# moddyz/stereo-to-multiview-cuda

Hardware: AMD Instinct MI355X
Metric: stereo->8-view frames/sec @1080p d=64; cost-agg HBM GB/s vs roofline (higher is better)
Workload: dtype f32; 1 GPU; 1920x1080 synthetic stereo frame, D=64, zd=32, full stereo->8-view frame: cost init + cross aggregation + WTA + DCC/IRV x5/bilateral + 6 DIBR views + interlacing, one frame per GPU per step; stages=3, usd=34, lsd=17, views=8, aggregation=matrix pipe (stm_kernels_aggm.hip)

## Files before the change

### stereo-to-multiview-cuda_amd/csrc/stm_kernels_aggm.hip

```cpp
#include "stm_hwin.h"

namespace stm {

typedef float f4 __attribute__((ext_vector_type(4)));

#define STM_MFMA16(m, b, acc, abid) __builtin_amdgcn_mfma_f32_16x16x1f32(m, b, acc, 2, abid, 0)
typedef float f16v __attribute__((ext_vector_type(16)));
typedef uint32_t u4v __attribute__((ext_vector_type(4)));
#define STM_MASKF(m) (__builtin_amdgcn_inverse_ballot_w64(m) ? 1.0f : 0.0f)
#define STM_BLOAD(rsrc, voff) __builtin_bit_cast(f4, __builtin_amdgcn_raw_buffer_load_b128(rsrc, voff, 0, 2))


template <int N> __device__ __forceinline__ float row_ror_f(float v)
{
    return __builtin_bit_cast(float, __builtin_amdgcn_update_dpp(0, __builtin_bit_cast(int, v), 0x120 + N, 0xf, 0xf, false));
}
template <int N> __device__ __forceinline__ int row_ror_i(int v) { return __builtin_amdgcn_update_dpp(0, v, 0x120 + N, 0xf, 0xf, false); }
__device__ __forceinline__ int wave_min_i(int v)
{
    v = min(v, row_ror_i<8>(v)); v = min(v, row_ror_i<4>(v)); v = min(v, row_ror_i<2>(v)); v = min(v, row_ror_i<1>(v));
    return min(min(__builtin_amdgcn_readlane(v, 0), __builtin_amdgcn_readlane(v, 16)),
               min(__builtin_amdgcn_readlane(v, 32), __builtin_amdgcn_readlane(v, 48)));
}
__device__ __forceinline__ int wave_max_i(int v)
// ... 370 lines not shown
                }
                int it = 1;
                for (; it + 2 <= n_it; it += 2) {
                    STM_HS_NEXT(ca)
                    STM_HS_MFMA(cb)
                    STM_HS_NEXT(cb)
                    STM_HS_MFMA(ca)
                }
                if (it < n_it) STM_HS_MFMA(cb)
#undef STM_HS_NEXT
#undef STM_HS_MFMA
            } else {
#pragma unroll
                for (int i = 0; i < 16; ++i) acc[i] = 0.f;
            }
            if (!WTA) {
#pragma unroll
                for (int cl = 0; cl < 4; ++cl) {
                    const f4 o = {acc[4 * cl], acc[4 * cl + 1], acc[4 * cl + 2], acc[4 * cl + 3]};
                    STM_BSTORE(rout[cl], (X0 >> 2) * 256 + l * 16, o);
                }
            } else {
                float bc[4];
                int bd[4];
#pragma unroll
                for (int i = 0; i < 4; ++i) { bc[i] = 3.402823466e+38f; bd[i] = 0; }
#pragma unroll
                for (int cl = 0; cl < 4; ++cl) {
                    const int d = (c0 + cl) * 16 + dd;
                    if (d < D) {
#pragma unroll
                        for (int i = 0; i < 4; ++i)
                            if (bc[i] > acc[4 * cl + i]) { bc[i] = acc[4 * cl + i]; bd[i] = d; }
                    }
                }
                const __amdgpu_buffer_rsrc_t rs = __builtin_amdgcn_make_buffer_rsrc((void *)(disp + row), 0, (uint32_t)W * 4u, 0x00020000);
#pragma unroll
                for (int i = 0; i < 4; ++i) {
                    const int bi = __builtin_bit_cast(int, bc[i]);
                    int m = bi;
                    m = min(m, row_ror_i<8>(m));
                    m = min(m, row_ror_i<4>(m));
                    m = min(m, row_ror_i<2>(m));
                    m = min(m, row_ror_i<1>(m));
                    int cand = (bi == m) ? bd[i] : 0x7fffffff;
                    cand = min(cand, row_ror_i<8>(cand));
                    cand = min(cand, row_ror_i<4>(cand));
                    cand = min(cand, row_ror_i<2>(cand));
                    cand = min(cand, row_ror_i<1>(cand));
                    if (ncs > 1) {
                        uint2 *slot = wb + (X0 - seg0 * TX + 4 * lb + i);
                        if (dd == 0) {
                            if (cs > 0) {
                                const uint2 pv = *slot;
                                if (!(m < (int)pv.x)) { m = (int)pv.x; cand = (int)pv.y; }
                            }
                            if (cs + 1 < ncs) *slot = make_uint2((uint32_t)m, (uint32_t)cand);
                        }
                        if (cs + 1 < ncs) continue;
                    }
                    __builtin_amdgcn_raw_buffer_store_b32(__builtin_bit_cast(uint32_t, (float)cand - (float)zd), rs,
                                                          dd == 0 ? (X0 + 4 * lb + i) * 4 : (int)0x7ffffff0, 0, 0);
                }
            }
        }
        __syncthreads();
        if (more) {
            int sl = slot0 + w;
            if (sl >= NJ) sl -= NJ;
#pragma unroll
            for (int k = 0; k < KP; ++k) tile[(k * NJ + sl) * 64 + l] = st[k];
            STM_HS_SN(sq + 1)
            slot0 += NW;
            if (slot0 >= NJ) slot0 -= NJ;
        }
        __syncthreads();
    }
  }
#undef STM_HS_LOAD
#undef STM_HS_ARMS
#undef STM_HS_SN
}

template <int NW>
__global__ __launch_bounds__(64 * NW, (2 * NW) / 4) void stm_k_pq_hc(PQViews v, int D, int zd, int H, int W, int G, int NC, int HG, int nseg,
                                                                     int spl, const float *__restrict__ lut_g, int pad, int dbg)
{
    constexpr int NT = 64 * NW, TX = 16 * NW, NEWPX = 16 * NW;
    extern __shared__ f4 lds4[];
    const int NG = 4 * NW + 2 * HG, NJ = NG >> 2;
    f4 *tile = lds4;
    uint32_t *sn = (uint32_t *)(tile + 4 * NG * 16);
    int2 *sg = (int2 *)(sn + TX);
    const int SO = NEWPX + 2 * pad;
    uint2 *s_own = (uint2 *)(sg + NW), *s_oth = s_own + 2 * NEWPX;
    float *s_lut_ad = (float *)(s_oth + 2 * SO), *s_lut_c = s_lut_ad + 768;
    const int tid = threadIdx.x, l = tid & 63, w = __builtin_amdgcn_readfirstlane(tid >> 6);
    const int lb = l >> 4, dd = l & 15;
    const int part = blockIdx.x % spl, rest = blockIdx.x / spl, y = rest % H, view = rest / H;
    const int seg_per = (nseg + spl - 1) / spl, seg0 = part * seg_per, seg1 = min(nseg, seg0 + seg_per);
    if (seg0 >= seg1) return;
    f4 *__restrict__ out = (f4 *)(view ? v.b[1] : v.b[0]);
    const u8 *__restrict__ armL = view ? v.armL[1] : v.armL[0], *__restrict__ armR = view ? v.armR[1] : v.armR[0];
    const uint32_t *__restrict__ pk_own = view ? v.pk[1] : v.pk[0], *__restrict__ pk_oth = view ? v.pk[0] : v.pk[1];
    const uint32_t *__restrict__ cen_own = view ? v.cen[1] : v.cen[0], *__restrict__ cen_oth = view ? v.cen[0] : v.cen[1];
    const int sgn = view ? -1 : 1;
    const size_t row = (size_t)y * W;
    const uint32_t rowbytes = (uint32_t)G * 256u;
    for (int i = tid; i < 768 + 65; i += NT) s_lut_ad[i] = lut_g[i];
    uint2 so = make_uint2(0, 0), sx = make_uint2(0, 0);
    int aLn = 0, aRn = 0;
    f4 cst[4];
  const int ncs = (NC + 3) >> 2;
  for (int cs = 0; cs < ncs; ++cs) {
    const int c0 = 4 * cs;
    __amdgpu_buffer_rsrc_t rout[4];
#pragma unroll
    for (int cl = 0; cl < 4; ++cl)
        rout[cl] = __builtin_amdgcn_make_buffer_rsrc((void *)(out + ((size_t)min(c0 + cl, NC - 1) * H + y) * G * 16), 0, c0 + cl < NC ? rowbytes : 0u, 0x00020000);
#define STM_HC_FETCH(A0)                                                                           \
    {                                                                                              \
        const int x0_ = 4 * ((A0) - HG);                                                           \
        if (tid < NEWPX) {                                                                         \
            const int gx = min(max(x0_ + tid, 0), W - 1);                                          \
            so = make_uint2(pk_own[row + gx], cen_own[row + gx]);                                  \
        }                                                                                          \
        if (tid < SO) {                                                                            \
            const int gx = min(max(x0_ - pad + tid, 0), W - 1);                                    \
            sx = make_uint2(pk_oth[row + gx], cen_oth[row + gx]);                                  \
        }                                                                                          \
    }
#define STM_HC_STAGE(B)                                            \
    {                                                              \
        if (tid < NEWPX) s_own[(B) * NEWPX + tid] = so;            \
        if (tid < SO) s_oth[(B) * SO + tid] = sx;                  \
    }
#define STM_HC_COSTS(B, A0)                                                                                               \
    {                                                                                                                     \
        const int gi = 4 * w + lb, x0g = 4 * ((A0) - HG + gi);                                                            \
        const uint2 *own = s_own + (B) * NEWPX + gi * 4;                                                                  \
        const uint2 o0 = own[0], o1 = own[1], o2 = own[2], o3 = own[3];                                                   \
        const bool in0 = x0g >= 0 && x0g < W, in1 = x0g + 1 >= 0 && x0g + 1 < W, in2 = x0g + 2 >= 0 && x0g + 2 < W,       \
                   in3 = x0g + 3 >= 0 && x0g + 3 < W;                                                                     \
         \
         \
        _Pragma("unroll") for (int cl = 0; cl < 4; ++cl) {                                                                \
            f4 val = {0.f, 0.f, 0.f, 0.f};                                                                                \
            if (c0 + cl < NC) {                                                                              \
                const int d = (c0 + cl) * 16 + dd;                   \
                const uint2 *oth = s_oth + (B) * SO + gi * 4 + sgn * (d - zd) + pad;                                      \
                const uint2 q0 = oth[0], q1 = oth[1], q2 = oth[2], q3 = oth[3];                                           \
                const float a0 = s_lut_ad[__builtin_amdgcn_sad_u8(o0.x, q0.x, 0u)], c0 = s_lut_c[hamdist_q1(o0.y, q0.y)]; \
                const float a1 = s_lut_ad[__builtin_amdgcn_sad_u8(o1.x, q1.x, 0u)], c1 = s_lut_c[hamdist_q1(o1.y, q1.y)]; \
                const float a2 = s_lut_ad[__builtin_amdgcn_sad_u8(o2.x, q2.x, 0u)], c2 = s_lut_c[hamdist_q1(o2.y, q2.y)]; \
                const float a3 = s_lut_ad[__builtin_amdgcn_sad_u8(o3.x, q3.x, 0u)], c3 = s_lut_c[hamdist_q1(o3.y, q3.y)]; \
                const bool dok = d < D;                                                                                   \
                val.x = (in0 && dok) ? a0 + c0 : 0.f;                                                                     \
                val.y = (in1 && dok) ? a1 + c1 : 0.f;                                                                     \
                val.z = (in2 && dok) ? a2 + c2 : 0.f;                                                                     \
                val.w = (in3 && dok) ? a3 + c3 : 0.f;                                                                     \
            }                                                                                                             \
            cst[cl] = val;                                                                                                \
        }                                                                                                                 \
    }
#define STM_HC_ARMS(S)                                                          \
    if (tid < TX) {                                                             \
        const int x = min((S) * TX + tid, W - 1);                               \
        aLn = armL[row + x];                                                    \
        aRn = armR[row + x];                                                    \
    }
#define STM_HC_SN(S)                                                                                                       \
    if (tid < TX) {                                                                                                        \
        const int x = (S) * TX + tid, org = (S) * TX - 4 * HG;                                                             \
         \
        const int srel_ = x < W ? x - aLn - org : x - org, nn_ = x < W ? aLn + aRn : 0;                                    \
        sn[tid] = (uint32_t)srel_ | ((uint32_t)nn_ << 16);                                                                 \
                           \
        int lo_ = nn_ ? (srel_ >> 2) : 0x7fffffff, hi_ = nn_ ? ((srel_ + nn_ + 3) >> 2) : -0x7fffffff;                     \
        lo_ = min(lo_, row_ror_i<8>(lo_)); lo_ = min(lo_, row_ror_i<4>(lo_)); lo_ = min(lo_, row_ror_i<2>(lo_)); lo_ = min(lo_, row_ror_i<1>(lo_)); \
        hi_ = max(hi_, row_ror_i<8>(hi_)); hi_ = max(hi_, row_ror_i<4>(hi_)); hi_ = max(hi_, row_ror_i<2>(hi_)); hi_ = max(hi_, row_ror_i<1>(hi_)); \
        if ((tid & 15) == 0) sg[tid >> 4] = make_int2(lo_, hi_ - lo_);                                                     \
    }
    for (int r0 = 0; r0 < NJ; r0 += NW) {
        const int a0 = 4 * NW * seg0 + 4 * r0;
        STM_HC_FETCH(a0)
        __syncthreads();
        STM_HC_STAGE(0)
        __syncthreads();
        if (r0 + w < NJ) {
            STM_HC_COSTS(0, a0)
#pragma unroll
            for (int k = 0; k < 4; ++k) tile[(k * NJ + (NW * seg0 + r0 + w) % NJ) * 64 + l] = cst[k];
        }
    }
    __syncthreads();
    {
        const int a1 = 4 * NW * (seg0 + 1) + NG - 4 * NW;
        STM_HC_FETCH(a1)
        STM_HC_STAGE((seg0 + 1) & 1)
        STM_HC_ARMS(seg0)
        STM_HC_SN(seg0)
    }
    __syncthreads();
    int slot0 = (NW * seg0) % NJ;
    for (int sq = seg0; sq < seg1; ++sq) {
        const int X0 = sq * TX + 16 * w;
        const bool more = sq + 1 < seg1;
        if (more) {
            STM_HC_FETCH(4 * NW * (sq + 2) + NG - 4 * NW)
            STM_HC_ARMS(sq + 1)
        }
        if (X0 < W) {
            const uint32_t e = sn[16 * w + dd];
            const int srel = (int)(e & 0xffffu), nn = (int)(e >> 16);
            const int2 sgw = sg[w];
            const int G0r = __builtin_amdgcn_readfirstlane(sgw.x);
            const int n_it = STM_DBG(dbg, 1) ? 0 : __builtin_amdgcn_readfirstlane(sgw.y);
            f16v acc;
            if (n_it > 0) {
                int gs = 4 * slot0 + G0r;
                if (gs >= NG) gs -= NG;
                const f4 *p = tile + (lb * NG + gs) * 16 + dd;
                int t = 4 * G0r + lb - srel;
#define STM_HS_NEXT(C)                                        \
    {                                                         \
        C = *p;                                               \
        p += 16;                                              \
        if (++gs == NG) { gs = 0; p -= NG * 16; }  \
    }
#define STM_HS_MFMA(C)                                                          \
    {                                                                           \
        const float m = ((unsigned)t < (unsigned)nn) ? 1.0f : 0.0f;             \
        t += 4;                                                                 \
        acc = STM_MFMA16(m, C.x, acc, 0);                                       \
        acc = STM_MFMA16(m, C.y, acc, 1);                                       \
        acc = STM_MFMA16(m, C.z, acc, 2);                                       \
        acc = STM_MFMA16(m, C.w, acc, 3);                                       \
    }
                f4 ca, cb;
                STM_HS_NEXT(ca)
                STM_HS_NEXT(cb)
                {
                    const float m = ((unsigned)t < (unsigned)nn) ? 1.0f : 0.0f;
                    t += 4;
                    const f16v z = {0.f, 0.f, 0.f, 0.f, 0.f, 0.f, 0.f, 0.f, 0.f, 0.f, 0.f, 0.f, 0.f, 0.f, 0.f, 0.f};
                    acc = STM_MFMA16(m, ca.x, z, 0);
                    acc = STM_MFMA16(m, ca.y, acc, 1);
                    acc = STM_MFMA16(m, ca.z, acc, 2);
                    acc = STM_MFMA16(m, ca.w, acc, 3);
                }
                int it = 1;
                for (; it + 2 <= n_it; it += 2) {
                    STM_HS_NEXT(ca)
                    STM_HS_MFMA(cb)
                    STM_HS_NEXT(cb)
                    STM_HS_MFMA(ca)
                }
                if (it < n_it) STM_HS_MFMA(cb)
#undef STM_HS_NEXT
#undef STM_HS_MFMA
            } else {
#pragma unroll
                for (int i = 0; i < 16; ++i) acc[i] = 0.f;
            }
#pragma unroll
            for (int cl = 0; cl < 4; ++cl) {
                const f4 o = {acc[4 * cl], acc[4 * cl + 1], acc[4 * cl + 2], acc[4 * cl + 3]};
                if (!STM_DBG(dbg, 4)) STM_BSTORE(rout[cl], (X0 >> 2) * 256 + l * 16, o);
            }
        }
        if (more) STM_HC_COSTS((sq + 1) & 1, 4 * NW * (sq + 1) + NG - 4 * NW)
        __syncthreads();
        if (more) {
            int sl = slot0 + w;
            if (sl >= NJ) sl -= NJ;
#pragma unroll
            for (int k = 0; k < 4; ++k) tile[(k * NJ + sl) * 64 + l] = cst[k];
            STM_HC_STAGE(sq & 1)
            STM_HC_SN(sq + 1)
            slot0 += NW;
            if (slot0 >= NJ) slot0 -= NJ;
        }
        __syncthreads();
    }
  }
#undef STM_HC_FETCH
#undef STM_HC_STAGE
#undef STM_HC_COSTS
#undef STM_HC_ARMS
#undef STM_HC_SN
}

constexpr int VT_EV = 2 * 255 + 32;
__global__ __launch_bounds__(256) void stm_k_vwin_table(PQViews v, uint32_t *__restrict__ tab, int rec, int H, int W, int G, int nT, int top)
{
    __shared__ unsigned long long ev_all[4][VT_EV];
    const int l = threadIdx.x & 63, wv = threadIdx.x >> 6, g = blockIdx.x * 4 + wv, u = blockIdx.y, view = blockIdx.z;
    if (g >= G) return;
    unsigned long long *ev = ev_all[wv];
    const u8 *__restrict__ armU = view ? v.armU[1] : v.armU[0], *__restrict__ armD = view ? v.armD[1] : v.armD[0];
    const int b = l >> 4, i = l & 15, y = u * 16 + i, x = 4 * g + b;
    int s0 = 0, nn = 0;
    if (y < H && x < W) {
        const int aU = armU[(size_t)y * W + x], aD = armD[(size_t)y * W + x];
        s0 = y - aU;
        nn = aU + aD;
    }
    vwin_build(tab + ((size_t)(view * nT + u) * G + g) * rec, ev, u, top, s0, nn);
}

typedef __attribute__((address_space(4))) const uint32_t ctab32;
typedef __attribute__((address_space(4))) const unsigned long long ctab64;
struct V12Quad { f4 c; unsigned long long m0, m1, m2, m3; };
struct V12Sweep {
    const f4 *p;
    ctab64 *mk;
    int qs, n_it;
    V12Quad A;
};
#define STM_V12_LOAD(S, Q, RQ)                                                      \
    {                                                                               \
        Q.c = *S.p;                                                                 \
        Q.m0 = S.mk[0]; Q.m1 = S.mk[1]; Q.m2 = S.mk[2]; Q.m3 = S.mk[3];             \
        S.p += 64; S.mk += 4;                                                       \
        if (++S.qs == RQ) { S.qs = 0; S.p -= RQ * 64; }                \
        asm volatile("" ::: "memory"); __builtin_amdgcn_sched_barrier(0);           \
    }
#define STM_V12_ARRIVED(Q) __builtin_amdgcn_sched_barrier(0); asm volatile("" : : "v"(Q.c), "s"(Q.m0), "s"(Q.m1), "s"(Q.m2), "s"(Q.m3) : "memory");
#define STM_V12_MFMA(Q)                                                                                            \
    {                                                                                                              \
        float a0 = STM_MASKF(Q.m0), a1 = STM_MASKF(Q.m1), a2 = STM_MASKF(Q.m2), a3 = STM_MASKF(Q.m3);              \
        asm volatile("" : "+v"(a0), "+v"(a1), "+v"(a2), "+v"(a3));  \
        acc = __builtin_amdgcn_mfma_f32_16x16x1f32(a0, Q.c.x, acc, 0, 0, 0);                                       \
        acc = __builtin_amdgcn_mfma_f32_16x16x1f32(a1, Q.c.y, acc, 0, 0, 0);                                       \
        acc = __builtin_amdgcn_mfma_f32_16x16x1f32(a2, Q.c.z, acc, 0, 0, 0);                                       \
        acc = __builtin_amdgcn_mfma_f32_16x16x1f32(a3, Q.c.w, acc, 0, 0, 0);                                       \
    }
__device__ __forceinline__ void v12t_begin(V12Sweep &S, const f4 *ring_l, int RQ, int slot0, int u4, ctab32 *r, int K0, int n_it)
{
    int qs = slot0 + ((K0 >> 2) - u4);
    if (qs < 0) qs += RQ;
    if (qs >= RQ) qs -= RQ;
    S.qs = qs;
    S.n_it = n_it;
    S.p = ring_l + qs * 64;
    S.mk = (ctab64 *)(r + 8);
    STM_V12_LOAD(S, S.A, RQ)
}
#define STM_V12_MFMA0(Q)                                                                                           \
    {                                                                                                              \
        float a0 = STM_MASKF(Q.m0), a1 = STM_MASKF(Q.m1), a2 = STM_MASKF(Q.m2), a3 = STM_MASKF(Q.m3);              \
        asm volatile("" : "+v"(a0), "+v"(a1), "+v"(a2), "+v"(a3));                                                 \
        const f16v z = {0.f, 0.f, 0.f, 0.f, 0.f, 0.f, 0.f, 0.f, 0.f, 0.f, 0.f, 0.f, 0.f, 0.f, 0.f, 0.f};           \
        acc = __builtin_amdgcn_mfma_f32_16x16x1f32(a0, Q.c.x, z, 0, 0, 0);                                         \
        acc = __builtin_amdgcn_mfma_f32_16x16x1f32(a1, Q.c.y, acc, 0, 0, 0);                                       \
        acc = __builtin_amdgcn_mfma_f32_16x16x1f32(a2, Q.c.z, acc, 0, 0, 0);                                       \
        acc = __builtin_amdgcn_mfma_f32_16x16x1f32(a3, Q.c.w, acc, 0, 0, 0);                                       \
    }
__device__ __forceinline__ f16v v12t_run(V12Sweep &S, int RQ)
{
    f16v acc;
    const int n_it = S.n_it;
    if (n_it == 0) {
#pragma unroll
        for (int i = 0; i < 16; ++i) acc[i] = 0.f;
        return acc;
    }
    V12Quad B;
    STM_V12_ARRIVED(S.A)
    STM_V12_LOAD(S, B, RQ)
    STM_V12_MFMA0(S.A)
    int it = 1;
    for (; it + 2 <= n_it; it += 2) {
// ... 147 lines not shown
static size_t v12t_smem(int usd)
{
    const int TS = 48, UQ = (usd + 3) & ~3, LAG = (UQ + TS - 1) / TS + 1;
    return (size_t)(TS + 2 * UQ + TS * (LAG + 1) + UQ) * 256;
}
bool aggm_supports(int usd, int H, int W)
{
    if (usd > 255) usd = 255;
    return usd >= 1 && v12t_smem(usd) <= 160 * 1024 && (unsigned long long)H * ((W + 3) / 4) * 256ull < (1ull << 31);
}

template <bool QUAD> __global__ __launch_bounds__(256) void stm_k_from_pq(const f4 *__restrict__ in, Vol out, int D, int H, int W, int G)
{
    const int t = blockIdx.x * 256 + threadIdx.x, y = blockIdx.y, c = blockIdx.z;
    const int g = t >> 2, q = 4 * c + (t & 3);
    if (g >= G || 4 * q >= D) return;
    const f4 *src = in + (((size_t)c * H + y) * G + g) * 16 + 4 * (t & 3);
    const f4 d0 = src[0], d1 = src[1], d2 = src[2], d3 = src[3];
#pragma unroll
    for (int k = 0; k < 4; ++k) {
        const int x = 4 * g + k;
        if (x < W) store_quad<QUAD, false>(out, q, D, (size_t)y * W + x, make_float4(d0[k], d1[k], d2[k], d3[k]));
    }
}
void launch_from_pq(const float *pq, Vol out, int D, int H, int W)
{
    const int G = (W + 3) / 4, NC = (D + 15) / 16;
    if (out.quad) STM_LAUNCH(stm_k_from_pq<true>, dim3(cdiv(4 * G, 256), H, NC), dim3(256), 0, stream(), (const f4 *)pq, out, D, H, W, G);
    else STM_LAUNCH(stm_k_from_pq<false>, dim3(cdiv(4 * G, 256), H, NC), dim3(256), 0, stream(), (const f4 *)pq, out, D, H, W, G);
    STM_CHECK_LAUNCH();
}

static void aggm_chain(PQViews &v, int nviews, bool from_costs, bool wta, const float *lut, int D, int zd, int H, int W, int usd,
                       uint32_t *htab_ready = nullptr, uint32_t *vtab_ready = nullptr)
{
    const int G = (W + 3) / 4, NC = (D + 15) / 16;
    if (usd > 255) usd = 255;
    constexpr int NW = 8;
    const int HG = ((usd + 3) / 4 + 2) & ~1, NG = 4 * NW + 2 * HG;
    const int nseg = cdiv(W, 16 * NW), nblk = ((nseg * H * nviews + 7) / 8) * 8;
    const size_t smem_h = (size_t)4 * NG * 256 + 16 * NW * 4;
    const int dbgh = timing_knobs();
    int pad = zd > D - 1 - zd ? zd : D - 1 - zd;
    pad = (pad < 0 ? 0 : pad) + 15;
    const size_t smem_cost = smem_h + (size_t)(4 * NG * 4 + 4 * pad + 768 + 72) * 4;
    const bool fuse_cost = from_costs && (agg_variant() / 1000000) % 10 != 1;
    const int spl = nseg > 24 ? cdiv(nseg, 16) : 1;
    const bool streaming = NG / 4 >= NW && (agg_variant() / 10) % 10 != 1 && (NC <= 4 || (agg_variant() / 10) % 10 != 2);
    constexpr int NTP = 3, TS = 16 * NTP;
    const int UQ = (usd + 3) & ~3, nT = (H + 15) / 16;
    const bool regs = aggv_supports(usd) && (agg_variant() / 10000000) % 10 != 1;
    const int rec = regs ? aggv_table_rec() : 8 + 8 * ((2 * usd + 21) / 4 + 2);
    const int LAG = (UQ + TS - 1) / TS + 1;
    const int RQ1 = (TS + 2 * UQ) / 4, RQ2 = (TS * (LAG + 1) + UQ) / 4;
    uint32_t *vtab = regs && vtab_ready ? vtab_ready : Workspace::get<uint32_t>((size_t)nviews * nT * G * rec);
    const bool hregs = wta && aggh_supports(usd, D) && (agg_variant() / 100000000) % 10 != 1;
    uint32_t *htab = !hregs ? nullptr : htab_ready ? htab_ready : Workspace::get<uint32_t>(aggh_table_dwords(nviews, H, W));
    {
        if (!(regs && vtab_ready)) {
            ProfScope p("pq_vtab");
            STM_LAUNCH(stm_k_vwin_table, dim3(cdiv(G, 4), nT, nviews), dim3(256), 0, stream(), v, vtab, rec, H, W, G, nT, regs ? aggv_table_top() : -1);
            STM_CHECK_LAUNCH();
        }
        if (hregs && !htab_ready) {
            ProfScope p("pq_htab");
            launch_hwin_table(v, nviews, htab, H, W);
        }
    }
    if (from_costs && !fuse_cost) {
        ProfScope p("pq_cost");
        const size_t smem = (size_t)(2 * PC_TX + 2 * (PC_TX + 2 * pad) + 768 + 72) * 4;
        allow_lds_m((const void *)stm_k_pq_cost, smem);
        STM_LAUNCH(stm_k_pq_cost, dim3(cdiv(W, PC_TX), H, nviews), dim3(PC_TX), smem, stream(), v, lut, D, zd, H, W, G, NC, pad);
        STM_CHECK_LAUNCH();
    }
    {
        ProfScope p("pq_h");
        constexpr int NWC = 12;
        const int NGc = 4 * NWC + 2 * HG;
        const size_t smem_c12 = (size_t)4 * NGc * 256 + 16 * NWC * 4 + (size_t)(4 * NGc * 4 + 4 * pad + 768 + 72) * 4;
        const size_t smem_hc = (size_t)4 * NGc * 256 + 16 * NWC * 4 + 8 * NWC + (size_t)(2 * 16 * NWC + 2 * (16 * NWC + 2 * pad)) * 8 + (768 + 72) * 4;
        const int nsegc = cdiv(W, 16 * NWC);
        const size_t smem_hc8 = (size_t)4 * NG * 256 + 16 * NW * 4 + 8 * NW + (size_t)(2 * 16 * NW + 2 * (16 * NW + 2 * pad)) * 8 + (768 + 72) * 4;
        const bool hc_ok = fuse_cost && (agg_variant() / 1000) % 10 == 0 && (NC <= 4 || (agg_variant() / 10) % 10 != 2);
        if (hc_ok && smem_hc <= 80 * 1024 && 16 * NWC + 2 * pad <= 64 * NWC) {
            const int splc = nsegc > 24 ? cdiv(nsegc, 16) : 1;
            allow_lds_m((const void *)stm_k_pq_hc<NWC>, smem_hc);
            STM_LAUNCH((stm_k_pq_hc<NWC>), dim3(nviews * H * splc), dim3(64 * NWC), smem_hc, stream(), v, D, zd, H, W, G, NC, HG, nsegc, splc, lut, pad, dbgh);
        } else if (hc_ok && smem_hc8 <= 80 * 1024 && 16 * NW + 2 * pad <= 64 * NW) {
            allow_lds_m((const void *)stm_k_pq_hc<NW>, smem_hc8);
            STM_LAUNCH((stm_k_pq_hc<NW>), dim3(nviews * H * spl), dim3(64 * NW), smem_hc8, stream(), v, D, zd, H, W, G, NC, HG, nseg, spl, lut, pad, dbgh);
        } else if (fuse_cost && smem_c12 <= 80 * 1024 && (agg_variant() / 1000) % 10 != 1) {
            const int nblkc = ((nsegc * H * nviews + 7) / 8) * 8;
            allow_lds_m((const void *)stm_k_pq_h<NWC, false, true>, smem_c12);
            STM_LAUNCH((stm_k_pq_h<NWC, false, true>), dim3(nblkc), dim3(64 * NWC), smem_c12, stream(), v, D, zd, H, W, G, NC, HG, nsegc, dbgh, lut, pad, nviews);
        } else if (fuse_cost) {
            allow_lds_m((const void *)stm_k_pq_h<NW, false, true>, smem_cost);
            STM_LAUNCH((stm_k_pq_h<NW, false, true>), dim3(nblk), dim3(64 * NW), smem_cost, stream(), v, D, zd, H, W, G, NC, HG, nseg, dbgh, lut, pad, nviews);
        } else if (streaming) {
            allow_lds_m((const void *)stm_k_pq_hs<NW, false>, smem_h);
            STM_LAUNCH((stm_k_pq_hs<NW, false>), dim3(nviews * H * spl), dim3(64 * NW), smem_h, stream(), v, D, zd, H, W, G, NC, HG, nseg, spl, dbgh);
        } else {
            allow_lds_m((const void *)stm_k_pq_h<NW, false, false>, smem_h);
            STM_LAUNCH((stm_k_pq_h<NW, false, false>), dim3(nblk), dim3(64 * NW), smem_h, stream(), v, D, zd, H, W, G, NC, HG, nseg, dbgh, lut, 0, nviews);
        }
        STM_CHECK_LAUNCH();
    }
    {
        ProfScope p("pq_v12");
        if (regs) {
            launch_pq_v12r(v, nviews, vtab, rec, H, W, G, NC);
        } else {
            const size_t smem = (size_t)(RQ1 + RQ2) * 1024;
            allow_lds_m((const void *)stm_k_pq_v12t<NTP>, smem);
            STM_LAUNCH(stm_k_pq_v12t<NTP>, dim3(G, NC, nviews), dim3(128 * NTP), smem, stream(), v, vtab, rec, H, W, G, NC, UQ, RQ1, RQ2, LAG, dbgh);
            STM_CHECK_LAUNCH();
        }
    }
    {
        ProfScope p("pq_hw");
        if (hregs) {
            launch_pq_hsr(v, nviews, htab, D, zd, H, W);
        } else if (streaming && !wta) {
            allow_lds_m((const void *)stm_k_pq_hs<NW, false>, smem_h);
            STM_LAUNCH((stm_k_pq_hs<NW, false>), dim3(nviews * H * spl), dim3(64 * NW), smem_h, stream(), v, D, zd, H, W, G, NC, HG, nseg, spl, dbgh);
        } else if (streaming) {
            const int splw = NC > 4 ? std::max(spl, cdiv(nseg * 16 * NW, 1920)) : spl;
            const size_t smem_w = smem_h + (NC > 4 ? (size_t)cdiv(nseg, splw) * 16 * NW * 8 : 0);
            allow_lds_m((const void *)stm_k_pq_hs<NW, true>, smem_w);
            STM_LAUNCH((stm_k_pq_hs<NW, true>), dim3(nviews * H * splw), dim3(64 * NW), smem_w, stream(), v, D, zd, H, W, G, NC, HG, nseg, splw, dbgh);
        } else if (!wta) {
            allow_lds_m((const void *)stm_k_pq_h<NW, false, false>, smem_h);
            STM_LAUNCH((stm_k_pq_h<NW, false, false>), dim3(nblk), dim3(64 * NW), smem_h, stream(), v, D, zd, H, W, G, NC, HG, nseg, dbgh, lut, 0, nviews);
        } else {
            allow_lds_m((const void *)stm_k_pq_h<NW, true, false>, smem_h);
            STM_LAUNCH((stm_k_pq_h<NW, true, false>), dim3(nblk), dim3(64 * NW), smem_h, stream(), v, D, zd, H, W, G, NC, HG, nseg, dbgh, lut, 0, nviews);
        }
        STM_CHECK_LAUNCH();
    }
}

size_t aggm_frame_vtab_dwords(int H, int W, int usd, int *rec, int *top)
{
    if (usd > 255) usd = 255;
    const bool regs = aggv_supports(usd) && (agg_variant() / 10000000) % 10 != 1;
    *rec = regs ? aggv_table_rec() : 0;
    *top = regs ? aggv_table_top() : -1;
    if (!regs || (agg_variant() / 1000000000) % 10 == 1) return 0;
    return (size_t)2 * ((H + 15) / 16) * ((W + 3) / 4) * *rec;
}
size_t aggm_frame_htab_dwords(int D, int H, int W, int usd, bool keep_volume)
{
    if (usd > 255) usd = 255;
    const bool hregs = !keep_volume && aggh_supports(usd, D) && (agg_variant() / 100000000) % 10 != 1;
    return hregs && (agg_variant() / 1000000000) % 10 != 1 ? aggh_table_dwords(2, H, W) : 0;
}
void launch_aggm_frame(const uint32_t *const *pk, const uint32_t *const *cen, const float *lut, float *const *vol_a, float *const *vol_b,
                       const u8 *const *armU, const u8 *const *armD, const u8 *const *armL, const u8 *const *armR, float *const *disp,
                       int D, int zd, int H, int W, int usd, bool keep_volume, uint32_t *htab_ready, uint32_t *vtab_ready)
{
    PQViews v;
    for (int i = 0; i < 2; ++i) {
        v.pk[i] = pk[i]; v.cen[i] = cen[i]; v.a[i] = vol_a[i]; v.b[i] = vol_b[i];
        v.armU[i] = armU[i]; v.armD[i] = armD[i]; v.armL[i] = armL[i]; v.armR[i] = armR[i]; v.disp[i] = disp[i];
    }
    aggm_chain(v, 2, true, !keep_volume, lut, D, zd, H, W, usd, htab_ready, vtab_ready);
}

static int vtab_rec(int usd)
{
    if (usd > 255) usd = 255;
    const bool regs = aggv_supports(usd) && (agg_variant() / 10000000) % 10 != 1;
    return regs ? aggv_table_rec() : 8 + 8 * ((2 * usd + 21) / 4 + 2);
}
// ... 29 lines not shown
```

Measured before the change: 624.2 frames/s.

## Share fused cost ring between left and right views in horizontal aggregation

Adds a kernel that computes matching costs once per row into a circular LDS ring buffer and runs both the left- and right-view horizontal cross aggregations from it. The right view reads the same costs at disparity-shifted offsets, so one block per row handles both views. This halves the cost computation and the pk/census loads compared with launching a block per view. In exchange it needs a much larger LDS allocation (up to 160 KB), which lowers occupancy, and it adds ring-wraparound indexing. It is taken by default when nviews==2, NC<=4 and the ring fits.

```diff
diff --git a/stereo-to-multiview-cuda_amd/csrc/stm_kernels_aggm.hip b/stereo-to-multiview-cuda_amd/csrc/stm_kernels_aggm.hip
--- a/stereo-to-multiview-cuda_amd/csrc/stm_kernels_aggm.hip
+++ b/stereo-to-multiview-cuda_amd/csrc/stm_kernels_aggm.hip
@@ -683,6 +683,242 @@
 #undef STM_HC_COSTS
 #undef STM_HC_ARMS
 #undef STM_HC_SN
+}
+
+constexpr int HC2_RP = 512;
+template <int NW>
+__global__ __launch_bounds__(64 * NW, NW / 4) void stm_k_pq_hc2(PQViews v, int D, int zd, int H, int W, int G, int NC, int HG, int nseg, int spl,
+                                                                const float *__restrict__ lut_g, int pad, int EXL, int EXR)
+{
+    constexpr int NT = 64 * NW, TX = 16 * NW, RP = HC2_RP;
+    extern __shared__ f4 lds4[];
+    float *ring = (float *)lds4;
+    uint32_t *sn = (uint32_t *)(ring + (RP + 4) * 64);
+    int2 *sg = (int2 *)(sn + 2 * TX);
+    const int SO = TX + 2 * pad;
+    uint2 *s_own = (uint2 *)(sg + 2 * NW), *s_oth = s_own + 2 * TX;
+    float *s_lut_ad = (float *)(s_oth + 2 * SO), *s_lut_c = s_lut_ad + 768;
+    const int tid = threadIdx.x, l = tid & 63, w = __builtin_amdgcn_readfirstlane(tid >> 6);
+    const int lb = l >> 4, dd = l & 15;
+    const int part = blockIdx.x % spl, y = blockIdx.x / spl;
+    const int seg_per = (nseg + spl - 1) / spl, seg0 = part * seg_per, seg1 = min(nseg, seg0 + seg_per);
+    if (seg0 >= seg1) return;
+    const int ROFF = 4 * HG + EXL, RN = TX + 8 * HG + EXL + EXR;
+    const int dl = min(l, 16 * NC - 1);
+    const bool dok = l < D;
+    const int vw = tid >= TX ? 1 : 0, tv = tid - vw * TX;
+    const u8 *__restrict__ armLv = vw ? v.armL[1] : v.armL[0], *__restrict__ armRv = vw ? v.armR[1] : v.armR[0];
+    const uint32_t *__restrict__ pkL = v.pk[0], *__restrict__ pkR = v.pk[1], *__restrict__ cenL = v.cen[0], *__restrict__ cenR = v.cen[1];
+    const size_t row = (size_t)y * W;
+    const uint32_t rowbytes = (uint32_t)G * 256u;
+    for (int i = tid; i < 768 + 65; i += NT) s_lut_ad[i] = lut_g[i];
+    __amdgpu_buffer_rsrc_t rout[2][4];
+#pragma unroll
+    for (int vv = 0; vv < 2; ++vv)
+#pragma unroll
+        for (int cl = 0; cl < 4; ++cl)
+            rout[vv][cl] = __builtin_amdgcn_make_buffer_rsrc((void *)((f4 *)(vv ? v.b[1] : v.b[0]) + ((size_t)min(cl, NC - 1) * H + y) * G * 16), 0,
+                                                             cl < NC ? rowbytes : 0u, 0x00020000);
+    uint2 so = make_uint2(0, 0), sx = make_uint2(0, 0);
+    int aLn = 0, aRn = 0;
+    f4 cst[4];
+#define STM_HC2_FETCH(P0)                                                                          \
+    {                                                                                              \
+        const int p0_ = (P0);                                                                      \
+        if (tid < TX) {                                                                            \
+            const int gx = min(max(p0_ + tid, 0), W - 1);                                          \
+            so = make_uint2(pkL[row + gx], cenL[row + gx]);                                        \
+        }                                                                                          \
+        if (tid < SO) {                                                                            \
+            const int gx = min(max(p0_ - pad + tid, 0), W - 1);                                    \
+            sx = make_uint2(pkR[row + gx], cenR[row + gx]);                                        \
+        }                                                                                          \
+    }
+#define STM_HC2_STAGE(B)                                           \
+    {                                                              \
+        if (tid < TX) s_own[(B) * TX + tid] = so;                  \
+        if (tid < SO) s_oth[(B) * SO + tid] = sx;                  \
+    }
+#define STM_HC2_COSTS(B)                                                                                                  \
+    {                                                                                                                     \
+        _Pragma("unroll") for (int k = 0; k < 4; ++k) {                                                                   \
+            const uint2 *own = s_own + (B) * TX + 16 * w + 4 * k;                                                         \
+            const uint2 o0 = own[0], o1 = own[1], o2 = own[2], o3 = own[3];                                               \
+            const uint2 *oth = s_oth + (B) * SO + 16 * w + 4 * k + dl - zd + pad;                                         \
+            const uint2 q0 = oth[0], q1 = oth[1], q2 = oth[2], q3 = oth[3];                                               \
+            const float a0 = s_lut_ad[__builtin_amdgcn_sad_u8(o0.x, q0.x, 0u)], c0 = s_lut_c[hamdist_q1(o0.y, q0.y)];     \
+            const float a1 = s_lut_ad[__builtin_amdgcn_sad_u8(o1.x, q1.x, 0u)], c1 = s_lut_c[hamdist_q1(o1.y, q1.y)];     \
+            const float a2 = s_lut_ad[__builtin_amdgcn_sad_u8(o2.x, q2.x, 0u)], c2 = s_lut_c[hamdist_q1(o2.y, q2.y)];     \
+            const float a3 = s_lut_ad[__builtin_amdgcn_sad_u8(o3.x, q3.x, 0u)], c3 = s_lut_c[hamdist_q1(o3.y, q3.y)];     \
+            cst[k].x = dok ? a0 + c0 : 0.f;                                                                               \
+            cst[k].y = dok ? a1 + c1 : 0.f;                                                                               \
+            cst[k].z = dok ? a2 + c2 : 0.f;                                                                               \
+            cst[k].w = dok ? a3 + c3 : 0.f;                                                                               \
+        }                                                                                                                 \
+    }
+#define STM_HC2_WRITE(P0, NV)                                                                      \
+    {                                                                                              \
+        _Pragma("unroll") for (int k = 0; k < 4; ++k) {                                            \
+            if (16 * w + 4 * k < (NV)) {                                              \
+                const int rpix = ((P0) + 16 * w + 4 * k + ROFF) & (RP - 1);                        \
+                float *dst = ring + rpix * 64 + l;                                                 \
+                dst[0] = cst[k].x; dst[64] = cst[k].y; dst[128] = cst[k].z; dst[192] = cst[k].w;   \
+                if (rpix == 0) {                                                                   \
+                    dst[RP * 64] = cst[k].x; dst[RP * 64 + 64] = cst[k].y; dst[RP * 64 + 128] = cst[k].z; \
+                }                                                                                  \
+            }                                                                                      \
+        }                                                                                          \
+    }
+#define STM_HC2_ARMS(S)                                                         \
+    if (tid < 2 * TX) {                                                         \
+        const int x = min((S) * TX + tv, W - 1);                                \
+        aLn = armLv[row + x];                                                   \
+        aRn = armRv[row + x];                                                   \
+    }
+#define STM_HC2_SN(S)                                                                                                      \
+    if (tid < 2 * TX) {                                                                                                    \
+        const int x = (S) * TX + tv, org = (S) * TX - 4 * HG;                                                              \
+         \
+        const int srel_ = x < W ? x - aLn - org : x - org, nn_ = x < W ? aLn + aRn : 0;                                    \
+        sn[tid] = (uint32_t)srel_ | ((uint32_t)nn_ << 16);                                                                 \
+                           \
+        int lo_ = nn_ ? (srel_ >> 2) : 0x7fffffff, hi_ = nn_ ? ((srel_ + nn_ + 3) >> 2) : -0x7fffffff;                     \
+        lo_ = min(lo_, row_ror_i<8>(lo_)); lo_ = min(lo_, row_ror_i<4>(lo_)); lo_ = min(lo_, row_ror_i<2>(lo_)); lo_ = min(lo_, row_ror_i<1>(lo_)); \
+        hi_ = max(hi_, row_ror_i<8>(hi_)); hi_ = max(hi_, row_ror_i<4>(hi_)); hi_ = max(hi_, row_ror_i<2>(hi_)); hi_ = max(hi_, row_ror_i<1>(hi_)); \
+        if ((tid & 15) == 0) sg[tid >> 4] = make_int2(lo_, hi_ - lo_);                                                     \
+    }
+    const int pbeg = seg0 * TX - ROFF;
+    for (int r0 = 0; r0 < RN; r0 += TX) {
+        STM_HC2_FETCH(pbeg + r0)
+        __syncthreads();
+        STM_HC2_STAGE(0)
+        __syncthreads();
+        STM_HC2_COSTS(0)
+        STM_HC2_WRITE(pbeg + r0, RN - r0)
+    }
+    __syncthreads();
+#define STM_HC2_PNEW(S) (((S) - 1) * TX - ROFF + RN)
+    {
+        STM_HC2_FETCH(STM_HC2_PNEW(seg0 + 1))
+        STM_HC2_STAGE((seg0 + 1) & 1)
+        STM_HC2_ARMS(seg0)
+        STM_HC2_SN(seg0)
+    }
+    __syncthreads();
+    const float *ringl = ring + l;
+    for (int sq = seg0; sq < seg1; ++sq) {
+        const int X0 = sq * TX + 16 * w;
+        const bool more = sq + 1 < seg1;
+        if (more) {
+            STM_HC2_FETCH(STM_HC2_PNEW(sq + 2))
+            STM_HC2_ARMS(sq + 1)
+        }
+        if (X0 < W) {
+#define STM_HS_MFMA(C)                                                          \
+    {                                                                           \
+        const float m = ((unsigned)t < (unsigned)nn) ? 1.0f : 0.0f;             \
+        t += 4;                                                                 \
+        acc = STM_MFMA16(m, C.x, acc, 0);                                       \
+        acc = STM_MFMA16(m, C.y, acc, 1);                                       \
+        acc = STM_MFMA16(m, C.z, acc, 2);                                       \
+        acc = STM_MFMA16(m, C.w, acc, 3);                                       \
+    }
+#define STM_HC2_SWEEP(VV)                                                                                                  \
+    {                                                                                                                      \
+        f4 ca, cb;                                                                                                         \
+        STM_HS_NEXT(ca)                                                                                                    \
+        STM_HS_NEXT(cb)                               \
+        {                        \
+            const float m = ((unsigned)t < (unsigned)nn) ? 1.0f : 0.0f;                                                    \
+            t += 4;                                                                                                        \
+            const f16v z = {0.f, 0.f, 0.f, 0.f, 0.f, 0.f, 0.f, 0.f, 0.f, 0.f, 0.f, 0.f, 0.f, 0.f, 0.f, 0.f};               \
+            acc = STM_MFMA16(m, ca.x, z, 0);                                                                               \
+            acc = STM_MFMA16(m, ca.y, acc, 1);                                                                             \
+            acc = STM_MFMA16(m, ca.z, acc, 2);                                                                             \
+            acc = STM_MFMA16(m, ca.w, acc, 3);                                                                             \
+        }                                                                                                                  \
+        int it = 1;                                                                                                        \
+        for (; it + 2 <= n_it; it += 2) {                                                                                  \
+            STM_HS_NEXT(ca)                                                                                                \
+            STM_HS_MFMA(cb)                                                                                                \
+            STM_HS_NEXT(cb)                          \
+            STM_HS_MFMA(ca)                                                                                                \
+        }                                                                                                                  \
+        if (it < n_it) STM_HS_MFMA(cb)                                                                                     \
+    }
+#define STM_HC2_STORE(VV)                                                                                                  \
+    _Pragma("unroll") for (int cl = 0; cl < 4; ++cl) {  \
+        const f4 o = {acc[4 * cl], acc[4 * cl + 1], acc[4 * cl + 2], acc[4 * cl + 3]};                                     \
+        STM_BSTORE(rout[VV][cl], (X0 >> 2) * 256 + l * 16, o);                                                             \
+    }
+            {
+                const uint32_t e = sn[16 * w + dd];
+                const int srel = (int)(e & 0xffffu), nn = (int)(e >> 16);
+                const int2 sgw = sg[w];
+                const int G0r = __builtin_amdgcn_readfirstlane(sgw.x);
+                const int n_it = __builtin_amdgcn_readfirstlane(sgw.y);
+                f16v acc;
+                if (n_it > 0) {
+                    int ri = (sq * TX + 4 * G0r + EXL) & (RP - 1);
+                    int t = 4 * G0r + lb - srel;
+#define STM_HS_NEXT(C)                                                                  \
+    {                                                                                   \
+        const float *p_ = ringl + ri * 64;                                              \
+        C.x = p_[0]; C.y = p_[64]; C.z = p_[128]; C.w = p_[192];                        \
+        ri = (ri + 4) & (RP - 1);                                                       \
+    }
+                    STM_HC2_SWEEP(0)
+#undef STM_HS_NEXT
+                } else {
+#pragma unroll
+                    for (int i = 0; i < 16; ++i) acc[i] = 0.f;
+                }
+                STM_HC2_STORE(0)
+            }
+            {
+                const uint32_t e = sn[TX + 16 * w + dd];
+                const int srel = (int)(e & 0xffffu), nn = (int)(e >> 16);
+                const int2 sgw = sg[NW + w];
+                const int G0r = __builtin_amdgcn_readfirstlane(sgw.x);
+                const int n_it = __builtin_amdgcn_readfirstlane(sgw.y);
+                f16v acc;
+                if (n_it > 0) {
+                    uint32_t ab = ((uint32_t)((sq * TX + 4 * G0r + EXL - (dl - zd)) & (RP - 1)) << 8) | ((uint32_t)l << 2);
+                    int t = 4 * G0r + lb - srel;
+#define STM_HS_NEXT(C)                                                                  \
+    {                                                                                   \
+        const float *p_ = (const float *)((const char *)ring + ab);                     \
+        C.x = p_[0]; C.y = p_[64]; C.z = p_[128]; C.w = p_[192];                        \
+        ab = (ab + 1024u) & (uint32_t)(RP * 256 - 1);                                   \
+    }
+                    STM_HC2_SWEEP(1)
+#undef STM_HS_NEXT
+                } else {
+#pragma unroll
+                    for (int i = 0; i < 16; ++i) acc[i] = 0.f;
+                }
+                STM_HC2_STORE(1)
+            }
+#undef STM_HS_MFMA
+#undef STM_HC2_SWEEP
+#undef STM_HC2_STORE
+        }
+        if (more) STM_HC2_COSTS((sq + 1) & 1)
+        __syncthreads();
+        if (more) {
+            STM_HC2_WRITE(STM_HC2_PNEW(sq + 1), TX)
+            STM_HC2_STAGE(sq & 1)
+            STM_HC2_SN(sq + 1)
+        }
+        __syncthreads();
+    }
+#undef STM_HC2_FETCH
+#undef STM_HC2_STAGE
+#undef STM_HC2_COSTS
+#undef STM_HC2_WRITE
+#undef STM_HC2_ARMS
+#undef STM_HC2_SN
+#undef STM_HC2_PNEW
 }
 
 constexpr int VT_EV = 2 * 255 + 32;
@@ -996,8 +1232,18 @@
         const size_t smem_hc = (size_t)4 * NGc * 256 + 16 * NWC * 4 + 8 * NWC + (size_t)(2 * 16 * NWC + 2 * (16 * NWC + 2 * pad)) * 8 + (768 + 72) * 4;
         const int nsegc = cdiv(W, 16 * NWC);
         const size_t smem_hc8 = (size_t)4 * NG * 256 + 16 * NW * 4 + 8 * NW + (size_t)(2 * 16 * NW + 2 * (16 * NW + 2 * pad)) * 8 + (768 + 72) * 4;
-        const bool hc_ok = fuse_cost && (agg_variant() / 1000) % 10 == 0 && (NC <= 4 || (agg_variant() / 10) % 10 != 2);
-        if (hc_ok && smem_hc <= 80 * 1024 && 16 * NWC + 2 * pad <= 64 * NWC) {
+        const int hv = (agg_variant() / 1000) % 10;
+        const bool hc_ok = fuse_cost && (hv == 0 || hv == 3) && (NC <= 4 || (agg_variant() / 10) % 10 != 2);
+        const int exl = (std::max(16 * NC - 1 - zd, 0) + 3) & ~3, exr = (std::max(zd, 0) + 3) & ~3;
+        const size_t smem_hc2 = (size_t)(HC2_RP + 4) * 256 + 2 * 16 * NWC * 4 + 2 * NWC * 8 + (size_t)(2 * 16 * NWC + 2 * (16 * NWC + 2 * pad)) * 8 + (768 + 72) * 4;
+        const bool hc2_ok = hc_ok && hv != 3 && nviews == 2 && NC <= 4 && zd >= 0 && 16 * NWC + 2 * pad <= 64 * NWC &&
+                            16 * NWC + 8 * HG + exl + exr <= HC2_RP && smem_hc2 <= 160 * 1024;
+        if (hc2_ok) {
+            ProfScope ps("hc_shared");
+            const int splc = nsegc > 24 ? cdiv(nsegc, 16) : 1;
+            allow_lds_m((const void *)stm_k_pq_hc2<NWC>, smem_hc2);
+            STM_LAUNCH((stm_k_pq_hc2<NWC>), dim3(H * splc), dim3(64 * NWC), smem_hc2, stream(), v, D, zd, H, W, G, NC, HG, nsegc, splc, lut, pad, exl, exr);
+        } else if (hc_ok && smem_hc <= 80 * 1024 && 16 * NWC + 2 * pad <= 64 * NWC) {
             const int splc = nsegc > 24 ? cdiv(nsegc, 16) : 1;
             allow_lds_m((const void *)stm_k_pq_hc<NWC>, smem_hc);
             STM_LAUNCH((stm_k_pq_hc<NWC>), dim3(nviews * H * splc), dim3(64 * NWC), smem_hc, stream(), v, D, zd, H, W, G, NC, HG, nsegc, splc, lut, pad, dbgh);
```

Measured after the change: 620.8 frames/s. No clear change (-0.5%).

## Specialize fused cost+horizontal-agg kernel with interior fast path and direct LDS addressing

Applied to the files above, without the earlier changes.

Splits the fused cost/horizontal aggregation kernel body into a template with a PARENT flag. The default variant gets an interior-tile cost path that skips per-pixel bounds checks and reads the LUTs through raw LDS addresses. The Hamming-LUT lookup is folded into popcount plus a bit offset. The MFMA feed loop now walks the ring-buffer tile pointer directly instead of going through the generic next macro. The old behaviour stays reachable as a selectable variant (hcv==3), at the cost of more code paths and address-space casts that depend on LUT layout assumptions.

```diff
diff --git a/stereo-to-multiview-cuda_amd/csrc/stm_kernels_aggm.hip b/stereo-to-multiview-cuda_amd/csrc/stm_kernels_aggm.hip
--- a/stereo-to-multiview-cuda_amd/csrc/stm_kernels_aggm.hip
+++ b/stereo-to-multiview-cuda_amd/csrc/stm_kernels_aggm.hip
@@ -476,9 +476,22 @@
 #undef STM_HS_SN
 }
 
-template <int NW>
-__global__ __launch_bounds__(64 * NW, (2 * NW) / 4) void stm_k_pq_hc(PQViews v, int D, int zd, int H, int W, int G, int NC, int HG, int nseg,
-                                                                     int spl, const float *__restrict__ lut_g, int pad, int dbg)
+typedef __attribute__((address_space(3))) const float hc_lds_cf;
+typedef uint32_t hc_u2 __attribute__((ext_vector_type(2)));
+typedef __attribute__((address_space(3))) const hc_u2 hc_lds_u2;
+__device__ __forceinline__ float hc_rho_c(uint32_t a, uint32_t b, uint32_t tab4)
+{
+    const uint32_t x = a ^ b;
+    return *(hc_lds_cf *)(uintptr_t)((((uint32_t)__popc(x) + tab4) << 2) + ((x >> 24) & 0x80u));
+}
+__device__ __forceinline__ float hc_rho_ad(uint32_t a, uint32_t b, uint32_t tab)
+{
+    return *(hc_lds_cf *)(uintptr_t)((__builtin_amdgcn_sad_u8(a, b, 0u) << 2) + tab);
+}
+
+template <int NW, bool PARENT>
+__device__ __forceinline__ void pq_hc_body(const PQViews &v, int D, int zd, int H, int W, int G, int NC, int HG, int nseg, int spl,
+                                           const float *__restrict__ lut_g, int pad, int dbg)
 {
     constexpr int NT = 64 * NW, TX = 16 * NW, NEWPX = 16 * NW;
     extern __shared__ f4 lds4[];
@@ -502,6 +515,8 @@
     const size_t row = (size_t)y * W;
     const uint32_t rowbytes = (uint32_t)G * 256u;
     for (int i = tid; i < 768 + 65; i += NT) s_lut_ad[i] = lut_g[i];
+    const uint32_t ad_lds = (uint32_t)(uintptr_t)(__attribute__((address_space(3))) float *)s_lut_ad;
+    const uint32_t c_lds4 = (uint32_t)(uintptr_t)(__attribute__((address_space(3))) float *)s_lut_c >> 2;
     uint2 so = make_uint2(0, 0), sx = make_uint2(0, 0);
     int aLn = 0, aRn = 0;
     f4 cst[4];
@@ -529,21 +544,21 @@
         if (tid < NEWPX) s_own[(B) * NEWPX + tid] = so;            \
         if (tid < SO) s_oth[(B) * SO + tid] = sx;                  \
     }
-#define STM_HC_COSTS(B, A0)                                                                                               \
+#define STM_HC_OTH(B)                                                                                                     \
+    const int d = (c0 + cl) * 16 + dd;                               \
+    const uint2 *oth = s_oth + (B) * SO + gi * 4 + sgn * (d - zd) + pad;                                                  \
+    const uint2 q0 = oth[0], q1 = oth[1], q2 = oth[2], q3 = oth[3];
+#define STM_HC_COSTS_EDGE(B, A0)                                                                                          \
     {                                                                                                                     \
         const int gi = 4 * w + lb, x0g = 4 * ((A0) - HG + gi);                                                            \
         const uint2 *own = s_own + (B) * NEWPX + gi * 4;                                                                  \
         const uint2 o0 = own[0], o1 = own[1], o2 = own[2], o3 = own[3];                                                   \
         const bool in0 = x0g >= 0 && x0g < W, in1 = x0g + 1 >= 0 && x0g + 1 < W, in2 = x0g + 2 >= 0 && x0g + 2 < W,       \
                    in3 = x0g + 3 >= 0 && x0g + 3 < W;                                                                     \
-         \
-         \
         _Pragma("unroll") for (int cl = 0; cl < 4; ++cl) {                                                                \
             f4 val = {0.f, 0.f, 0.f, 0.f};                                                                                \
             if (c0 + cl < NC) {                                                                              \
-                const int d = (c0 + cl) * 16 + dd;                   \
-                const uint2 *oth = s_oth + (B) * SO + gi * 4 + sgn * (d - zd) + pad;                                      \
-                const uint2 q0 = oth[0], q1 = oth[1], q2 = oth[2], q3 = oth[3];                                           \
+                STM_HC_OTH(B)                                                                                             \
                 const float a0 = s_lut_ad[__builtin_amdgcn_sad_u8(o0.x, q0.x, 0u)], c0 = s_lut_c[hamdist_q1(o0.y, q0.y)]; \
                 const float a1 = s_lut_ad[__builtin_amdgcn_sad_u8(o1.x, q1.x, 0u)], c1 = s_lut_c[hamdist_q1(o1.y, q1.y)]; \
                 const float a2 = s_lut_ad[__builtin_amdgcn_sad_u8(o2.x, q2.x, 0u)], c2 = s_lut_c[hamdist_q1(o2.y, q2.y)]; \
@@ -556,6 +571,48 @@
             }                                                                                                             \
             cst[cl] = val;                                                                                                \
         }                                                                                                                 \
+    }
+#define STM_HC_SUMS(CL)                                                                                                   \
+    {                                                                                                                     \
+         \
+        hc_lds_u2 *oth = (hc_lds_u2 *)(uintptr_t)(oth0 + (uint32_t)((CL) * 128 * sgn));                                   \
+        const hc_u2 q0 = oth[0], q1 = oth[1], q2 = oth[2], q3 = oth[3];                                                   \
+        cst[CL].x = hc_rho_ad(o0.x, q0.x, ad_lds) + hc_rho_c(o0.y, q0.y, c_lds4);                                         \
+        cst[CL].y = hc_rho_ad(o1.x, q1.x, ad_lds) + hc_rho_c(o1.y, q1.y, c_lds4);                                         \
+        cst[CL].z = hc_rho_ad(o2.x, q2.x, ad_lds) + hc_rho_c(o2.y, q2.y, c_lds4);                                         \
+        cst[CL].w = hc_rho_ad(o3.x, q3.x, ad_lds) + hc_rho_c(o3.y, q3.y, c_lds4);                                         \
+    }
+#define STM_HC_COSTS_IN(B, A0)                                                                                            \
+    {                                                                                                                     \
+        const int gi = 4 * w + lb;                                                                                        \
+        const uint2 *own = s_own + (B) * NEWPX + gi * 4;                                                                  \
+        const uint2 o0 = own[0], o1 = own[1], o2 = own[2], o3 = own[3];                                                   \
+         \
+         \
+        uint32_t oth0 = (uint32_t)(uintptr_t)(hc_lds_u2 *)(s_oth + (B) * SO + gi * 4 + sgn * (c0 * 16 + dd - zd) + pad); \
+        asm("" : "+v"(oth0));                                                                                             \
+        if ((c0 + 4) * 16 <= D) {                                       \
+            STM_HC_SUMS(0) STM_HC_SUMS(1) STM_HC_SUMS(2) STM_HC_SUMS(3)                                                   \
+        } else {                                                                                                          \
+            _Pragma("unroll") for (int cl = 0; cl < 4; ++cl) {                                                            \
+                if (c0 + cl < NC) {                                                                          \
+                    STM_HC_SUMS(cl)                                                                                       \
+                    if ((c0 + cl) * 16 + 16 > D) {                                        \
+                        const bool dok = (c0 + cl) * 16 + dd < D;                                                         \
+                        cst[cl].x = dok ? cst[cl].x : 0.f; cst[cl].y = dok ? cst[cl].y : 0.f;                             \
+                        cst[cl].z = dok ? cst[cl].z : 0.f; cst[cl].w = dok ? cst[cl].w : 0.f;                             \
+                    }                                                                                                     \
+                } else {                                                                                                  \
+                    cst[cl] = f4{0.f, 0.f, 0.f, 0.f};                                                                     \
+                }                                                                                                         \
+            }                                                                                                             \
+        }                                                                                                                 \
+    }
+#define STM_HC_COSTS(B, A0)                                                                                               \
+    {                                                                                                                     \
+        const int xw_ = 4 * ((A0) - HG + 4 * w);                           \
+        if (!PARENT && xw_ >= 0 && xw_ + 16 <= W) STM_HC_COSTS_IN(B, A0)                                                  \
+        else STM_HC_COSTS_EDGE(B, A0)                                                                                     \
     }
 #define STM_HC_ARMS(S)                                                          \
     if (tid < TX) {                                                             \
@@ -631,28 +688,62 @@
         acc = STM_MFMA16(m, C.z, acc, 2);                                       \
         acc = STM_MFMA16(m, C.w, acc, 3);                                       \
     }
+#define STM_HS_MFMA0(C)                                                         \
+    {                                                                           \
+        const float m = ((unsigned)t < (unsigned)nn) ? 1.0f : 0.0f;             \
+        t += 4;                                                                 \
+        const f16v z = {0.f, 0.f, 0.f, 0.f, 0.f, 0.f, 0.f, 0.f, 0.f, 0.f, 0.f, 0.f, 0.f, 0.f, 0.f, 0.f}; \
+        acc = STM_MFMA16(m, C.x, z, 0);                                         \
+        acc = STM_MFMA16(m, C.y, acc, 1);                                       \
+        acc = STM_MFMA16(m, C.z, acc, 2);                                       \
+        acc = STM_MFMA16(m, C.w, acc, 3);                                       \
+    }
                 f4 ca, cb;
-                STM_HS_NEXT(ca)
-                STM_HS_NEXT(cb)
-                {
-                    const float m = ((unsigned)t < (unsigned)nn) ? 1.0f : 0.0f;
-                    t += 4;
-                    const f16v z = {0.f, 0.f, 0.f, 0.f, 0.f, 0.f, 0.f, 0.f, 0.f, 0.f, 0.f, 0.f, 0.f, 0.f, 0.f, 0.f};
-                    acc = STM_MFMA16(m, ca.x, z, 0);
-                    acc = STM_MFMA16(m, ca.y, acc, 1);
-                    acc = STM_MFMA16(m, ca.z, acc, 2);
-                    acc = STM_MFMA16(m, ca.w, acc, 3);
-                }
                 int it = 1;
-                for (; it + 2 <= n_it; it += 2) {
+                if (PARENT) {
                     STM_HS_NEXT(ca)
-                    STM_HS_MFMA(cb)
                     STM_HS_NEXT(cb)
-                    STM_HS_MFMA(ca)
+                    STM_HS_MFMA0(ca)
+                    for (; it + 2 <= n_it; it += 2) {
+                        STM_HS_NEXT(ca)
+                        STM_HS_MFMA(cb)
+                        STM_HS_NEXT(cb)
+                        STM_HS_MFMA(ca)
+                    }
+                } else {
+                    const int n1 = NG - gs, back = 32 - NG * 16;
+                    if (!(n1 & 1)) {
+                        const int itw = n1 - 3;
+                        ca = p[0];
+                        cb = p[16];
+                        p += n1 == 2 ? back : 32;
+                        STM_HS_MFMA0(ca)
+                        for (; it + 2 <= n_it; it += 2) {
+                            ca = p[0];
+                            STM_HS_MFMA(cb)
+                            cb = p[16];
+                            p += it == itw ? back : 32;
+                            STM_HS_MFMA(ca)
+                        }
+                    } else {
+                        const int itw = n1 - 2;
+                        ca = p[0];
+                        p += n1 == 1 ? 16 - NG * 16 : 16;
+                        cb = p[0];
+                        STM_HS_MFMA0(ca)
+                        for (; it + 2 <= n_it; it += 2) {
+                            ca = p[16];
+                            p += it == itw ? back : 32;
+                            STM_HS_MFMA(cb)
+                            cb = p[0];
+                            STM_HS_MFMA(ca)
+                        }
+                    }
                 }
                 if (it < n_it) STM_HS_MFMA(cb)
 #undef STM_HS_NEXT
 #undef STM_HS_MFMA
+#undef STM_HS_MFMA0
             } else {
 #pragma unroll
                 for (int i = 0; i < 16; ++i) acc[i] = 0.f;
@@ -680,9 +771,25 @@
   }
 #undef STM_HC_FETCH
 #undef STM_HC_STAGE
+#undef STM_HC_OTH
+#undef STM_HC_COSTS_EDGE
+#undef STM_HC_SUMS
+#undef STM_HC_COSTS_IN
 #undef STM_HC_COSTS
 #undef STM_HC_ARMS
 #undef STM_HC_SN
+}
+template <int NW>
+__global__ __launch_bounds__(64 * NW, (2 * NW) / 4) void stm_k_pq_hc(PQViews v, int D, int zd, int H, int W, int G, int NC, int HG, int nseg,
+                                                                     int spl, const float *__restrict__ lut_g, int pad, int dbg)
+{
+    pq_hc_body<NW, false>(v, D, zd, H, W, G, NC, HG, nseg, spl, lut_g, pad, dbg);
+}
+template <int NW>
+__global__ __launch_bounds__(64 * NW, (2 * NW) / 4) void stm_k_pq_hc_sel(PQViews v, int D, int zd, int H, int W, int G, int NC, int HG, int nseg,
+                                                                         int spl, const float *__restrict__ lut_g, int pad, int dbg)
+{
+    pq_hc_body<NW, true>(v, D, zd, H, W, G, NC, HG, nseg, spl, lut_g, pad, dbg);
 }
 
 constexpr int VT_EV = 2 * 255 + 32;
@@ -996,14 +1103,17 @@
         const size_t smem_hc = (size_t)4 * NGc * 256 + 16 * NWC * 4 + 8 * NWC + (size_t)(2 * 16 * NWC + 2 * (16 * NWC + 2 * pad)) * 8 + (768 + 72) * 4;
         const int nsegc = cdiv(W, 16 * NWC);
         const size_t smem_hc8 = (size_t)4 * NG * 256 + 16 * NW * 4 + 8 * NW + (size_t)(2 * 16 * NW + 2 * (16 * NW + 2 * pad)) * 8 + (768 + 72) * 4;
-        const bool hc_ok = fuse_cost && (agg_variant() / 1000) % 10 == 0 && (NC <= 4 || (agg_variant() / 10) % 10 != 2);
+        const int hcv = (agg_variant() / 1000) % 10;
+        const bool hc_ok = fuse_cost && (hcv == 0 || hcv == 3) && (NC <= 4 || (agg_variant() / 10) % 10 != 2);
         if (hc_ok && smem_hc <= 80 * 1024 && 16 * NWC + 2 * pad <= 64 * NWC) {
             const int splc = nsegc > 24 ? cdiv(nsegc, 16) : 1;
-            allow_lds_m((const void *)stm_k_pq_hc<NWC>, smem_hc);
-            STM_LAUNCH((stm_k_pq_hc<NWC>), dim3(nviews * H * splc), dim3(64 * NWC), smem_hc, stream(), v, D, zd, H, W, G, NC, HG, nsegc, splc, lut, pad, dbgh);
+            const auto k = hcv == 3 ? stm_k_pq_hc_sel<NWC> : stm_k_pq_hc<NWC>;
+            allow_lds_m((const void *)k, smem_hc);
+            STM_LAUNCH(k, dim3(nviews * H * splc), dim3(64 * NWC), smem_hc, stream(), v, D, zd, H, W, G, NC, HG, nsegc, splc, lut, pad, dbgh);
         } else if (hc_ok && smem_hc8 <= 80 * 1024 && 16 * NW + 2 * pad <= 64 * NW) {
-            allow_lds_m((const void *)stm_k_pq_hc<NW>, smem_hc8);
-            STM_LAUNCH((stm_k_pq_hc<NW>), dim3(nviews * H * spl), dim3(64 * NW), smem_hc8, stream(), v, D, zd, H, W, G, NC, HG, nseg, spl, lut, pad, dbgh);
+            const auto k = hcv == 3 ? stm_k_pq_hc_sel<NW> : stm_k_pq_hc<NW>;
+            allow_lds_m((const void *)k, smem_hc8);
+            STM_LAUNCH(k, dim3(nviews * H * spl), dim3(64 * NW), smem_hc8, stream(), v, D, zd, H, W, G, NC, HG, nseg, spl, lut, pad, dbgh);
         } else if (fuse_cost && smem_c12 <= 80 * 1024 && (agg_variant() / 1000) % 10 != 1) {
             const int nblkc = ((nsegc * H * nviews + 7) / 8) * 8;
             allow_lds_m((const void *)stm_k_pq_h<NWC, false, true>, smem_c12);
```

New measurement: 625.2 frames/s before, 624.6 frames/s after. Within noise of the previous version (-0.1%).
